# tsadja/ShaSTA

Hardware: AMD Instinct MI355X
Metric: affinity frame-pairs/sec at N=M=500, F=256 (higher is better)
Workload: dtype f32; 1 GPU; synthetic N=M=500, F=256 (num_point 4 x C 64), nf=7: affinity forward from HBM-resident NHWC BEV maps (SURVEY 8a rows 4-16); max_obj=500, num_feats=7, num_point=4, arithmetic=f16x2, parallelism=replica x1

## Files before the change

### shasta_amd/csrc/anchor_split.hip

```cpp
#include "stages.hpp"
#include "lds_dma.hpp"
#include "pieces.hpp"

#include <stdlib.h>

#include <type_traits>

namespace shasta {

struct RowMaxArgs {
    const float* base[4];
    long stride;
    int rows, len;
    unsigned* out;
    float* sumabs;
};
__global__ __launch_bounds__(256) void row_max_kernel(RowMaxArgs a) {
    __shared__ float red[4];
    const int row = blockIdx.y, src = blockIdx.z;
    const int n4 = a.len / 4, per = (n4 + gridDim.x - 1) / gridDim.x;
    const int beg = blockIdx.x * per, end = min(n4, beg + per);
    const f32x4* p = reinterpret_cast<const f32x4*>(a.base[src] + (size_t)row * a.stride);
    float m = 0.0f, sa = 0.0f;
    for (int i = beg + threadIdx.x; i < end; i += 256) {
        const f32x4 v = __builtin_nontemporal_load(p + i);
        m = fmaxf(fmaxf(m, fmaxf(fabsf(v[0]), fabsf(v[1]))), fmaxf(fabsf(v[2]), fabsf(v[3])));
        sa += (fabsf(v[0]) + fabsf(v[1])) + (fabsf(v[2]) + fabsf(v[3]));
    }
#pragma unroll
    for (int off = 32; off > 0; off >>= 1) m = fmaxf(m, __shfl_xor(m, off, 64));
    if ((threadIdx.x & 63) == 0) red[threadIdx.x >> 6] = m;
    __syncthreads();
    if (threadIdx.x == 0) atomicMax(a.out + src * a.rows + row, __float_as_uint(fmaxf(fmaxf(red[0], red[1]), fmaxf(red[2], red[3]))));
    if (a.sumabs) {
        sa = wave_sum(sa);
        if ((threadIdx.x & 63) == 0) atomicAdd(a.sumabs + src * a.rows + row, sa);
    }
}

__global__ __launch_bounds__(256) void aux_ratio_kernel(const unsigned* __restrict__ wmax, const float* __restrict__ sumabs, int rows, int K,
                                                        float* __restrict__ summary) {
    __shared__ float rbest[4];
    __shared__ int ibest[4];
    float best = 0.0f;
    int where = 0;
    for (int r = threadIdx.x; r < rows; r += 256) {
        const float mx = __uint_as_float(wmax[r]), sa = sumabs[r], rest = sa - mx;
        const float ratio = !(mx > 0.0f) || K < 2 ? (mx == mx ? 0.0f : mx) : rest > sa * 1e-6f ? mx * (float)(K - 1) / rest : INFINITY;
        if (!(ratio <= best)) {
            best = ratio;
            where = r;
        }
    }
#pragma unroll
    for (int off = 32; off > 0; off >>= 1) {
        const float ob = __shfl_xor(best, off, 64);
        const int ow = __shfl_xor(where, off, 64);
        if (!(ob <= best)) {
            best = ob;
            where = ow;
        }
    }
    if ((threadIdx.x & 63) == 0) {
        rbest[threadIdx.x >> 6] = best;
        ibest[threadIdx.x >> 6] = where;
    }
    __syncthreads();
    if (threadIdx.x == 0) {
        for (int w = 1; w < 4; ++w)
            if (!(rbest[w] <= best)) {
                best = rbest[w];
                where = ibest[w];
            }
        summary[0] = best;
        summary[1] = (float)where;
    }
}

static int row_max_chunks(int rows, int sources, int len) {
    int c = 1;
    while (c < 64 && rows * sources * c < 2048 && len / (c * 2) >= 4096) c *= 2;
    return c;
}
int launch_x_maxima(const float* feat, const float* prev_feat, int K, int B, int x_batch_stride, unsigned* xmax, hipStream_t st) {
    if (hipMemsetAsync(xmax, 0, (size_t)2 * B * sizeof(unsigned), st) != hipSuccess) return SHASTA_E_LAUNCH;
    RowMaxArgs r;
    r.base[0] = feat;
    r.base[1] = prev_feat;
    r.base[2] = r.base[3] = nullptr;
    r.stride = x_batch_stride;
    r.rows = B;
    r.len = K;
    r.out = xmax;
    r.sumabs = nullptr;
    hipLaunchKernelGGL(row_max_kernel, dim3(row_max_chunks(B, 2, K), B, 2), dim3(256), 0, st, r);
    return check_launch("row_max (activations)");
}
int launch_w_maxima(const float* const W[4], int H, int K, unsigned* wmax, float* sumabs, hipStream_t st) {
    if (hipMemsetAsync(wmax, 0, (size_t)4 * H * sizeof(unsigned), st) != hipSuccess) return SHASTA_E_LAUNCH;
    if (sumabs && hipMemsetAsync(sumabs, 0, ((size_t)4 * H + 16) * sizeof(float), st) != hipSuccess) return SHASTA_E_LAUNCH;
    RowMaxArgs r;
    for (int i = 0; i < 4; ++i) r.base[i] = W[i];
    r.stride = K;
    r.rows = H;
    r.len = K;
    r.out = wmax;
    r.sumabs = sumabs;
    hipLaunchKernelGGL(row_max_kernel, dim3(row_max_chunks(H, 4, K), H, 4), dim3(256), 0, st, r);
    int rc = check_launch("row_max (weights)");
    if (rc || !sumabs) return rc;
    hipLaunchKernelGGL(aux_ratio_kernel, dim3(1), dim3(256), 0, st, wmax, sumabs, 4 * H, K, sumabs + (size_t)4 * H);
    return check_launch("aux_ratio");
}



struct SplitXArgs {
    const float* x[2];
    uint32_t* xs;
    int B, KT, NBLK, XT, x_batch_stride, NP;
    const unsigned* xmax;
};

__global__ __launch_bounds__(256) void split_x_kernel(SplitXArgs a) {
    __shared__ __attribute__((aligned(16))) float tile[32][264];
    const int src = blockIdx.z, bblk = blockIdx.y / a.XT, u = blockIdx.y % a.XT;
    const int kt0 = blockIdx.x * 8, nkt = min(8, a.KT - kt0);
    const float* x = a.x[src];
    const int brow0 = (bblk * a.XT + u) * 32;
    for (int i = threadIdx.x; i < 32 * 64; i += 256) {
        const int r = i >> 6, c4 = i & 63, b = brow0 + r;
        f32x4 v = {0.0f, 0.0f, 0.0f, 0.0f};
        if (b < a.B && (c4 >> 3) < nkt)
            v = *reinterpret_cast<const f32x4*>(x + (size_t)b * a.x_batch_stride + (size_t)kt0 * 32 + c4 * 4);
        *reinterpret_cast<f32x4*>(&tile[r][c4 * 4]) = v;
    }
    __syncthreads();
    for (int i = threadIdx.x; i < 1024; i += 256) {
        const int lane = i & 63, s = (i >> 6) & 1, ktl = i >> 7;
        if (ktl >= nkt) continue;
        const int r = lane & 31, h = lane >> 5;
        const float* p = &tile[r][ktl * 32 + 16 * s + 8 * h];
        const f32x4 v0 = *reinterpret_cast<const f32x4*>(p), v1 = *reinterpret_cast<const f32x4*>(p + 4);
        const float v[8] = {v0[0], v0[1], v0[2], v0[3], v1[0], v1[1], v1[2], v1[3]};
        if (a.NP == 2) {
            const int e = range_exponent_bits(a.xmax[src * a.B + min(brow0 + r, a.B - 1)]);
            u32x4 hi, lo;
            cut2_f16x8([&](int j) { return v[j]; }, e, hi, lo);
            const size_t frag0 = ((((size_t)src * a.NBLK + bblk) * a.KT + kt0 + ktl) * (4 * a.XT)) + (size_t)(u * 2 + s) * 2;
            u32x4* o = reinterpret_cast<u32x4*>(a.xs) + frag0 * 64 + lane;
            o[0] = hi;
            o[64] = lo;
            continue;
        }
        u32x4 hi, mid, lo;
#pragma unroll
        for (int j = 0; j < 4; ++j) {
            float h0, m0, l0, h1, m1, l1;
            cut3_bf16(v[2 * j], h0, m0, l0);
            cut3_bf16(v[2 * j + 1], h1, m1, l1);
            hi[j] = pack_bf16x2(h0, h1);
            mid[j] = pack_bf16x2(m0, m1);
            lo[j] = pack_bf16x2(l0, l1);
        }
        const size_t frag0 = ((((size_t)src * a.NBLK + bblk) * a.KT + kt0 + ktl) * (6 * a.XT)) + (size_t)(u * 2 + s) * 3;
        u32x4* o = reinterpret_cast<u32x4*>(a.xs) + frag0 * 64 + lane;
        o[0] = hi;
        o[64] = mid;
        o[128] = lo;
    }
}

struct PrecutArgs {
    const float* W[4];
    const unsigned* wmax;
    uint32_t* img;
    int H, K, KT, G;
};
__global__ __launch_bounds__(256) void precut_weights_kernel(PrecutArgs a) {
    __shared__ __attribute__((aligned(16))) float tile[32][260];
    const int mlp = blockIdx.z, g = blockIdx.y, kt0 = blockIdx.x * 8, nkt = min(8, a.KT - kt0);
    const float* W = a.W[mlp];
    for (int i = threadIdx.x; i < 32 * 64; i += 256) {
        const int r = i >> 6, c4 = i & 63, row = g * 32 + r;
        f32x4 v = {0.0f, 0.0f, 0.0f, 0.0f};
        if (row < a.H && (c4 >> 3) < nkt) v = __builtin_nontemporal_load(reinterpret_cast<const f32x4*>(W + (size_t)row * a.K + (size_t)kt0 * 32) + c4);
        *reinterpret_cast<f32x4*>(&tile[r][c4 * 4]) = v;
    }
    __syncthreads();
    const int lane = threadIdx.x & 63;
    for (int f = threadIdx.x >> 6; f < 2 * nkt; f += 4) {
        const int ktl = f >> 1, sstep = f & 1;
        const int frow = lane & 31;
        const int wex = range_exponent_bits(a.wmax[mlp * a.H + min(g * 32 + frow, a.H - 1)]);
        const float* p = &tile[frow][ktl * 32 + 16 * sstep + 8 * (lane >> 5)];
        u32x4 hi, lo;
        cut2_f16x8([&](int j) { return p[j]; }, wex, hi, lo);
        u32x4* o = reinterpret_cast<u32x4*>(a.img) + ((((size_t)mlp * a.G + g) * a.KT + kt0 + ktl) * 4 + sstep * 2) * 64 + lane;
        o[0] = hi;
        o[64] = lo;
    }
}
size_t precut_image_bytes(int H, int K) { return (K % 32 != 0 || H == 0) ? 0 : (size_t)4 * cdiv(H, 32) * (K / 32) * 4096; }
int launch_precut_weights(const float* const W[4], const unsigned* wmax, void* img, int H, int K, hipStream_t st) {
    PrecutArgs a;
    for (int i = 0; i < 4; ++i) a.W[i] = W[i];
    a.wmax = wmax;
    a.img = static_cast<uint32_t*>(img);
    a.H = H;
    a.K = K;
    a.KT = K / 32;
    a.G = cdiv(H, 32);
    hipLaunchKernelGGL(precut_weights_kernel, dim3(cdiv(a.KT, 8), a.G, 4), dim3(256), 0, st, a);
    return check_launch("precut_weights");
}

struct AnchorSplitArgs {
    const uint32_t* wimg;
    const float* W[4];
    const uint32_t* xs;
    float* part;
    int H, K, B, KS, Kc, KT, NBLK, groups_per_mlp;
    const unsigned* wmax;
};

template <int XT, int NS, int NP, bool PRECUT = false>
__global__ __launch_bounds__(256) void anchor_l1_split_kernel(AnchorSplitArgs a) {
    static_assert(!PRECUT || NP == 2, "the pre-cut image holds fp16 pieces");
    constexpr int NPROD = NP == 3 ? 6 : 3;
    constexpr int XCH = 2 * NP * XT;
    constexpr int XPW = XCH / 4;
    static_assert(XCH % 4 == 0, "x fragments are dealt to four waves");
    constexpr int SLOT = 4 * 1024 + XCH * 256;
    constexpr int PER_TILE = 4 + XPW;
    static_assert(PER_TILE * (NS - 1) <= 63, "vmcnt is 6 bits");
    constexpr int NM = 2 * NPROD * XT;
    constexpr int ND = PER_TILE;
    constexpr int NR = 4 + XCH;
    constexpr int SG = PRECUT ? 1 : (NM - 8) / 16;
    constexpr int RPG = PRECUT ? (NR + NM - 2) / (NM - 1) : 1;
    static_assert(PRECUT ? (1 + (NR + RPG - 1) / RPG <= NM && 1 + ND <= NM) : (1 + NR < NM && 6 + 15 * SG < NM),
                  "side work must fit the MFMA gaps of one tile");
    extern __shared__ __attribute__((aligned(16))) float lds[];
    const int lane = threadIdx.x & 63;
    const int wid = __builtin_amdgcn_readfirstlane(threadIdx.x >> 6);

    const int ncombo = 2 * a.KS;
    const int combo = blockIdx.x % ncombo, rest = blockIdx.x / ncombo;
    const int quad = rest / a.NBLK;
    const int ks = combo >> 1, src = combo & 1;
    const int G2 = 2 * a.groups_per_mlp;
    const bool active = quad * 4 + wid < G2;
    const int gg = min(quad * 4 + wid, G2 - 1);
    const int mlp = 2 * src + gg / a.groups_per_mlp, r0 = (gg % a.groups_per_mlp) * 32;
    const int bblk = rest % a.NBLK;
    const int tpc = a.Kc >> 5;
    const int kt_beg = ks * tpc, NT = min(a.KT, kt_beg + tpc) - kt_beg;

    const float* wbase = mlp == 0 ? a.W[0] : mlp == 1 ? a.W[1] : mlp == 2 ? a.W[2] : a.W[3];
    const char* wub = PRECUT ? reinterpret_cast<const char*>(a.wimg) + (((size_t)mlp * a.groups_per_mlp + (r0 >> 5)) * a.KT + kt_beg) * 4096
                             : reinterpret_cast<const char*>(wbase + (size_t)r0 * a.K + (size_t)kt_beg * 32);
    const char* xub = reinterpret_cast<const char*>(a.xs) + ((((size_t)src * a.NBLK + bblk) * a.KT + kt_beg) * XCH) * 1024;
    uint32_t woff[4];
    {
        const int cpos = lane & 7, rl = lane >> 3;
#pragma unroll
        for (int j = 0; j < 4; ++j) {
            const int r = 8 * j + rl;
            const int c = cpos ^ ((r >> 1) & 7);
            woff[j] = (uint32_t)(((min(r0 + r, a.H - 1) - r0) * a.K + 4 * c) * 4);
        }
        if (PRECUT) woff[0] = (uint32_t)(lane * 16);
    }
    const uint32_t xoff = (uint32_t)(lane * 16 + wid * 1024);
    const uint32_t lds0 = (uint32_t)(size_t)((__attribute__((address_space(3))) float*)lds);
    auto dma = [&](int t, int slot, int idx) {
        if (idx < 4) {
            const char* base = PRECUT ? wub + (size_t)t * 4096 + (size_t)idx * 1024 : wub + (size_t)t * 128;
            const uint32_t dst = lds0 + (uint32_t)((slot * SLOT + wid * 1024 + idx * 256) * 4);
            lds_dma_x4_nt(PRECUT ? woff[0] : woff[idx], base, dst);
        } else {
            const int i = idx - 4;
            const char* base = xub + (size_t)t * (XCH * 1024) + (size_t)i * 4096;
            const uint32_t dst = lds0 + (uint32_t)((slot * SLOT + 4096 + (wid + 4 * i) * 256) * 4);
            lds_dma_x4(xoff, base, dst);
        }
    };
    auto issue = [&](int t, int slot) {
#pragma unroll
        for (int j = 0; j < ND; ++j) dma(t, slot, j);
    };

    struct Frag {
        u32x4 A[2][NP];
        u32x4 X[XT][2][NP];
    };
    f32x4 raw[4];
    const int frow = lane & 31, fh = lane >> 5, fsw = (frow >> 1) & 7;
    auto read_one = [&](int slot, Frag& f, int idx) {
        const float* sl = lds + slot * SLOT;
        if (idx < 4) {
            const int s = idx >> 1, qq = idx & 1;
            if constexpr (PRECUT) f.A[s][qq] = *reinterpret_cast<const u32x4*>(sl + wid * 1024 + idx * 256 + lane * 4);
            else raw[idx] = *reinterpret_cast<const f32x4*>(sl + wid * 1024 + frow * 32 + (((4 * s + 2 * fh + qq) ^ fsw) * 4));
        } else {
            const int j = idx - 4;
            f.X[j / (2 * NP)][(j / NP) % 2][j % NP] = *reinterpret_cast<const u32x4*>(sl + 4096 + j * 256 + lane * 4);
        }
    };
    float ph = 0.0f, pm = 0.0f, pl = 0.0f;
    _Float16 qh = 0, ql = 0;
    int wex = 0;
    if constexpr (NP == 2 && !PRECUT) wex = range_exponent_bits(a.wmax[mlp * a.H + min(r0 + frow, a.H - 1)]);
    auto cut_one = [&](Frag& f, int e) {
        if constexpr (PRECUT) return;
        const int s = e >> 3, d = (e & 7) >> 1;
        if constexpr (NP == 2) {
            _Float16 h, l;
            cut2_f16(__builtin_ldexpf(raw[e >> 2][e & 3], wex), h, l);
            if ((e & 1) == 0) {
                qh = h;
                ql = l;
            } else {
                f.A[s][0][d] = pack_f16x2(qh, h);
                f.A[s][1][d] = pack_f16x2(ql, l);
            }
        } else {
            float h, m, l;
            cut3_bf16(raw[e >> 2][e & 3], h, m, l);
            if ((e & 1) == 0) {
                ph = h;
                pm = m;
                pl = l;
            } else {
                f.A[s][0][d] = pack_bf16x2(ph, h);
                f.A[s][1][d] = pack_bf16x2(pm, m);
                f.A[s][NP - 1][d] = pack_bf16x2(pl, l);
            }
        }
    };

    f32x16 acc[XT];
#pragma unroll
    for (int u = 0; u < XT; ++u) acc[u] = f32x16{0, 0, 0, 0, 0, 0, 0, 0, 0, 0, 0, 0, 0, 0, 0, 0};
    auto mma_one = [&](const Frag& f, int i) {
        const int s = i / (NPROD * XT), u = (i / NPROD) % XT, pr = i % NPROD;
        if constexpr (NP == 3) acc[u] = mfma_32x32x16_bf16(f.A[s][kProductsBf16[pr].a], f.X[u][s][kProductsBf16[pr].b], acc[u]);
        else acc[u] = mfma_32x32x16_f16(f.A[s][kProductsF16[pr].a], f.X[u][s][kProductsF16[pr].b], acc[u]);
    };

    {
        int s = 0;
#pragma unroll 1
        for (int t = 0; t < NS && t < NT; ++t, ++s) issue(t, s);
    }
    Frag fa, fb;
    if (NT >= NS) wait_vmcnt<PER_TILE*(NS - 1)>();
    else wait_vmcnt<0>();
    __builtin_amdgcn_s_barrier();
    if (NT > 0) {
#pragma unroll
        for (int i = 0; i < NR; ++i) read_one(0, fa, i);
#pragma unroll
        for (int e = 0; e < 16; ++e) cut_one(fa, e);
    }
    auto step = [&](const Frag& cur, Frag& nxt, int t, int sc, auto steady) {
        constexpr bool STEADY = decltype(steady)::value;
        const int sn = sc + 1 == NS ? 0 : sc + 1;
#pragma unroll
        for (int i = 0; i < NM; ++i) {
            mma_one(cur, i);
            __builtin_amdgcn_sched_barrier(0);
            if (i == 0) {
                asm volatile("s_waitcnt lgkmcnt(0)" ::: "memory");
                if constexpr (STEADY) wait_vmcnt<PER_TILE*(NS - 2)>();
                else wait_vmcnt<0>();
                __builtin_amdgcn_s_barrier();
                if constexpr (!STEADY) {
                    if (t + NS < NT) issue(t + NS, sc);
                }
            }
            if (i >= 1 && i - 1 < ND) {
                if constexpr (STEADY) dma(t + NS, sc, i - 1);
            }
            if (i >= 1) {
#pragma unroll
                for (int r = 0; r < RPG; ++r)
                    if ((i - 1) * RPG + r < NR) read_one(sn, nxt, (i - 1) * RPG + r);
            }
            if constexpr (!PRECUT) {
                if (i >= 6 && (i - 6) % SG == 0 && (i - 6) / SG < 16) cut_one(nxt, (i - 6) / SG);
            }
            __builtin_amdgcn_sched_barrier(0);
        }
    };
    int t = 0, sc = 0;
    auto next = [&](int s) { return s + 1 == NS ? 0 : s + 1; };
#pragma unroll 1
    for (; t + NS + 1 < NT; t += 2) {
        step(fa, fb, t, sc, std::true_type{});
        sc = next(sc);
        step(fb, fa, t + 1, sc, std::true_type{});
        sc = next(sc);
    }
#pragma unroll 1
    for (; t + 1 < NT; t += 2) {
        step(fa, fb, t, sc, std::false_type{});
        sc = next(sc);
        step(fb, fa, t + 1, sc, std::false_type{});
        sc = next(sc);
    }
    if (t < NT) step(fa, fb, t, sc, std::false_type{});

    if (active) {
#pragma unroll
        for (int u = 0; u < XT; ++u) {
            const int b = (bblk * XT + u) * 32 + frow;
            if (b < a.B) {
                float* o = a.part + ((size_t)ks * a.B + b) * (4 * a.H) + mlp * a.H;
#pragma unroll
                for (int r = 0; r < 16; ++r) {
                    const int row = r0 + (r & 3) + 8 * (r >> 2) + 4 * fh;
                    if (row < a.H) o[row] = acc[u][r];
                }
            }
        }
    }
}

template <int NS>
__global__ __launch_bounds__(512) void anchor_l1_wide_kernel(AnchorSplitArgs a) {
    constexpr int XT = 16;
    constexpr int SLOT = (8 + 2 * XT) * 256;
    constexpr int ND = 5, NR = 12, NM = 24;
    static_assert(ND * (NS - 1) <= 63, "vmcnt is 6 bits");
    extern __shared__ __attribute__((aligned(16))) float lds[];
    const int lane = threadIdx.x & 63;
    const int wid = __builtin_amdgcn_readfirstlane(threadIdx.x >> 6);
    const int rg2 = wid & 1, ig = wid >> 1;

    const int ncombo = 2 * a.KS;
    const int combo = blockIdx.x % ncombo, rest = blockIdx.x / ncombo;
    const int quad = rest / a.NBLK, bblk = rest % a.NBLK;
    const int ks = combo >> 1, src = combo & 1;
    const int G2 = 2 * a.groups_per_mlp;
    const int tpc = a.Kc >> 5;
    const int kt_beg = ks * tpc, NT = 2 * (min(a.KT, kt_beg + tpc) - kt_beg);

    auto group_base = [&](int gq, int& mlp, int& r0) {
        const int gg = min(quad * 4 + gq, G2 - 1);
        mlp = 2 * src + gg / a.groups_per_mlp;
        r0 = (gg % a.groups_per_mlp) * 32;
    };
    int mlpw, r0w;
    group_base(wid >> 1, mlpw, r0w);
    const char* wub = reinterpret_cast<const char*>(a.wimg) + (((size_t)mlpw * a.groups_per_mlp + (r0w >> 5)) * a.KT + kt_beg) * 4096 + (wid & 1) * 1024;
    const char* xub = reinterpret_cast<const char*>(a.xs) + ((((size_t)src * a.NBLK + bblk) * a.KT + kt_beg) * (4 * XT)) * 1024;
    const uint32_t loff = (uint32_t)(lane * 16);
    const uint32_t lds0 = (uint32_t)(size_t)((__attribute__((address_space(3))) float*)lds);
    auto dma = [&](int t, int slot, int idx) {
        if (idx == 0) {
            const char* base = wub + (size_t)(t >> 1) * 4096 + (size_t)(t & 1) * 2048;
            const uint32_t dst = lds0 + (uint32_t)((slot * SLOT + wid * 256) * 4);
            lds_dma_x4(loff, base, dst);
        } else {
            const int f = 4 * wid + idx - 1, u = f >> 1, pc = f & 1;
            const char* base = xub + (size_t)(t >> 1) * (4 * XT * 1024) + (size_t)(((u * 2 + (t & 1)) * 2 + pc) * 1024);
            const uint32_t dst = lds0 + (uint32_t)((slot * SLOT + 2048 + f * 256) * 4);
            lds_dma_x4(loff, base, dst);
        }
    };
    struct Frag {
        u32x4 A[2][2];
        u32x4 X[4][2];
    };
    auto read_one = [&](int slot, Frag& f, int idx) {
        const float* sl = lds + slot * SLOT + lane * 4;
        if (idx < 4) f.A[idx >> 1][idx & 1] = *reinterpret_cast<const u32x4*>(sl + ((2 * rg2 + (idx >> 1)) * 2 + (idx & 1)) * 256);
        else f.X[(idx - 4) >> 1][idx & 1] = *reinterpret_cast<const u32x4*>(sl + 2048 + ((4 * ig + ((idx - 4) >> 1)) * 2 + (idx & 1)) * 256);
    };
    f32x16 acc[2][4];
#pragma unroll
    for (int j = 0; j < 2; ++j)
#pragma unroll
        for (int u = 0; u < 4; ++u) acc[j][u] = f32x16{0, 0, 0, 0, 0, 0, 0, 0, 0, 0, 0, 0, 0, 0, 0, 0};
    auto mma_one = [&](const Frag& f, int i) {
        const int pr = i >> 3, j = (i >> 2) & 1, u = i & 3;
        acc[j][u] = mfma_32x32x16_f16(f.A[j][kProductsF16[pr].a], f.X[u][kProductsF16[pr].b], acc[j][u]);
    };
    {
        int sl = 0;
#pragma unroll 1
        for (int t = 0; t < NS && t < NT; ++t, ++sl)
#pragma unroll
            for (int j = 0; j < ND; ++j) dma(t, sl, j);
    }
    Frag fa, fb;
    if (NT >= NS) wait_vmcnt<ND*(NS - 1)>();
    else wait_vmcnt<0>();
    __builtin_amdgcn_s_barrier();
    if (NT > 0) {
#pragma unroll
        for (int i = 0; i < NR; ++i) read_one(0, fa, i);
    }
    auto step = [&](const Frag& cur, Frag& nxt, int t, int sc, auto steady) {
        constexpr bool STEADY = decltype(steady)::value;
        const int sn = sc + 1 == NS ? 0 : sc + 1;
#pragma unroll
        for (int i = 0; i < NM; ++i) {
            mma_one(cur, i);
            __builtin_amdgcn_sched_barrier(0);
            if (i == 0) {
                asm volatile("s_waitcnt lgkmcnt(0)" ::: "memory");
                if constexpr (STEADY) wait_vmcnt<ND*(NS - 2)>();
                else wait_vmcnt<0>();
                __builtin_amdgcn_s_barrier();
                if constexpr (!STEADY) {
                    if (t + NS < NT) {
#pragma unroll
                        for (int j = 0; j < ND; ++j) dma(t + NS, sc, j);
                    }
                }
            }
            if (i >= 1 && i - 1 < ND) {
                if constexpr (STEADY) dma(t + NS, sc, i - 1);
            }
            if (i >= 1 && i - 1 < NR) read_one(sn, nxt, i - 1);
            __builtin_amdgcn_sched_barrier(0);
        }
    };
    int t = 0, sc = 0;
    auto next = [&](int s) { return s + 1 == NS ? 0 : s + 1; };
#pragma unroll 1
    for (; t + NS + 1 < NT; t += 2) {
        step(fa, fb, t, sc, std::true_type{});
        sc = next(sc);
        step(fb, fa, t + 1, sc, std::true_type{});
        sc = next(sc);
    }
#pragma unroll 1
    for (; t + 1 < NT; t += 2) {
        step(fa, fb, t, sc, std::false_type{});
        sc = next(sc);
        step(fb, fa, t + 1, sc, std::false_type{});
        sc = next(sc);
    }
    if (t < NT) step(fa, fb, t, sc, std::false_type{});
    const int frow = lane & 31, fh = lane >> 5;
#pragma unroll
    for (int j = 0; j < 2; ++j) {
        if (quad * 4 + 2 * rg2 + j >= G2) continue;
        int mlp, r0;
        group_base(2 * rg2 + j, mlp, r0);
#pragma unroll
        for (int u = 0; u < 4; ++u) {
            const int b = (bblk * XT + 4 * ig + u) * 32 + frow;
            if (b >= a.B) continue;
            float* o = a.part + ((size_t)ks * a.B + b) * (4 * a.H) + mlp * a.H;
#pragma unroll
            for (int r = 0; r < 16; ++r) {
                const int row = r0 + (r & 3) + 8 * (r >> 2) + 4 * fh;
                if (row < a.H) o[row] = acc[j][u][r];
            }
        }
    }
}

static inline bool split_wide(int B, int np, bool precut) { return np == 2 && precut && B > 256 && cdiv(B, 512) * 512 <= cdiv(B, 256) * 256; }

static inline int split_xt(int B, int np) { return np == 2 ? (B > 128 ? 8 : B > 64 ? 4 : B > 32 ? 2 : 1) : (B <= 64 ? 2 : 4); }
static inline int split_nblk(int B, int np) { return cdiv(B, 32 * split_xt(B, np)); }

size_t anchor_split_workspace_bytes(int B, int K) {
    if (B < 2 || K % 32 != 0) return 0;
    const size_t b3 = (size_t)2 * split_nblk(B, 3) * 32 * split_xt(B, 3) * (size_t)K * 6;
    const size_t b2 = (size_t)2 * split_nblk(B, 2) * 32 * split_xt(B, 2) * (size_t)K * 4;
    return align_up(b3 > b2 ? b3 : b2, 256);
}

bool anchor_split_serves(int B, int K, int x_batch_stride) { return B > 32 && K % 32 == 0 && (x_batch_stride & 3) == 0; }

void launch_split_x(const float* feat, const float* prev_feat, void* xs, int K, int B, int x_batch_stride, int np, const unsigned* xmax,
                    bool precut, hipStream_t st) {
    const bool wide = split_wide(B, np, precut);
    const int XT = wide ? 16 : split_xt(B, np), NBLK = wide ? cdiv(B, 512) : split_nblk(B, np), KT = K / 32;
    SplitXArgs sx;
    sx.x[0] = feat;
    sx.x[1] = prev_feat;
    sx.xs = static_cast<uint32_t*>(xs);
    sx.B = B;
    sx.KT = KT;
    sx.NBLK = NBLK;
    sx.XT = XT;
    sx.x_batch_stride = x_batch_stride;
    sx.NP = np;
    sx.xmax = xmax;
    hipLaunchKernelGGL(split_x_kernel, dim3(cdiv(KT, 8), NBLK * XT, 2), dim3(256), 0, st, sx);
}

void launch_anchor_l1_split(const float* const W[4], const void* xs, float* part, int H, int K, int B, int* ks_out, int np,
                            const unsigned* wmax, const void* wimg, hipStream_t st) {
    const bool wide = split_wide(B, np, wimg != nullptr);
    const int XT = wide ? 16 : split_xt(B, np), NBLK = wide ? cdiv(B, 512) : split_nblk(B, np), KT = K / 32;
    AnchorSplitArgs a;
    for (int i = 0; i < 4; ++i) a.W[i] = W[i];
    a.xs = static_cast<const uint32_t*>(xs);
    a.part = part;
    a.H = H;
    a.K = K;
    a.B = B;
    a.KT = KT;
    a.NBLK = NBLK;
    a.groups_per_mlp = cdiv(H, 32);
    a.wmax = wmax;
    a.wimg = static_cast<const uint32_t*>(wimg);
    const int quads = cdiv(2 * a.groups_per_mlp, 4);
    int ncu = 256;
    {
        int dev = 0;
        if (hipGetDevice(&dev) == hipSuccess) {
            int v = 0;
            if (hipDeviceGetAttribute(&v, hipDeviceAttributeMultiprocessorCount, dev) == hipSuccess && v > 0) ncu = v;
        }
    }
    const int cmin = KT >= 64 ? 4 : 1;
    int ks = cmin;
    double best = -1.0;
    const int nblk_split = split_nblk(B, np);
    for (int c = cmin; c <= 64 && c * 16 <= KT; ++c) {
        const int wgs = 2 * cdiv(KT, cdiv(KT, c)) * quads * nblk_split;
        const int rounds = cdiv(wgs, ncu);
        const double eff = (double)wgs / ((double)rounds * ncu);
        if (eff > best + 1e-9) {
            best = eff;
            ks = c;
        }
    }
    const int tiles_per = cdiv(KT, ks);
    a.Kc = tiles_per * 32;
    a.KS = cdiv(KT, tiles_per);
    *ks_out = a.KS;
    auto launch = [&](auto kern, int ns, int xt) {
        const size_t ldsb = (size_t)ns * (4 * 1024 + 2 * np * xt * 256) * sizeof(float);
        (void)hipFuncSetAttribute((const void*)kern, hipFuncAttributeMaxDynamicSharedMemorySize, (int)ldsb);
        hipLaunchKernelGGL(kern, dim3(2 * a.KS * quads * NBLK), dim3(256), ldsb, st, a);
    };
    if (wide) {
        const size_t ldsb = (size_t)4 * (8 + 2 * 16) * 1024;
        if (hipFuncSetAttribute((const void*)anchor_l1_wide_kernel<4>, hipFuncAttributeMaxDynamicSharedMemorySize, (int)ldsb) == hipSuccess) {
            hipLaunchKernelGGL(anchor_l1_wide_kernel<4>, dim3(2 * a.KS * quads * NBLK), dim3(512), ldsb, st, a);
        } else {
            (void)hipGetLastError();
            const size_t lds3 = (size_t)3 * (8 + 2 * 16) * 1024;
            (void)hipFuncSetAttribute((const void*)anchor_l1_wide_kernel<3>, hipFuncAttributeMaxDynamicSharedMemorySize, (int)lds3);
            hipLaunchKernelGGL(anchor_l1_wide_kernel<3>, dim3(2 * a.KS * quads * NBLK), dim3(512), lds3, st, a);
        }
    } else if (np == 2 && wimg) {
        if (XT == 1) launch(anchor_l1_split_kernel<1, 6, 2, true>, 6, 1);
        else if (XT == 2) launch(anchor_l1_split_kernel<2, 5, 2, true>, 5, 2);
        else if (XT == 4) launch(anchor_l1_split_kernel<4, 4, 2, true>, 4, 4);
        else launch(anchor_l1_split_kernel<8, 3, 2, true>, 3, 8);
    } else if (np == 2) {
        if (XT == 4) launch(anchor_l1_split_kernel<4, 4, 2>, 4, 4);
        else launch(anchor_l1_split_kernel<8, 3, 2>, 3, 8);
    } else if (XT == 2) launch(anchor_l1_split_kernel<2, 5, 3>, 5, 2);
    else launch(anchor_l1_split_kernel<4, 4, 3>, 4, 4);
}

}
```

Measured before the change: 64630 frame-pairs/s.

## Load activation fragments directly to registers in wide anchor kernel, stage only weights in LDS

The wide anchor layer-1 kernel previously staged both weight and activation tiles through LDS via DMA. Now each wave loads its own activation fragments straight from global memory into registers one step ahead, and only the shared weight tiles go through LDS. The wave-to-tile mapping changes from a 2x4 to a 4x2 accumulator layout, the LDS ring shrinks to 3 small slots, and the output store uses 16-byte vector writes when aligned. This cuts LDS footprint and LDS traffic, but exposes global-load latency directly to registers with only one step of prefetch and raises register pressure.

```diff
diff --git a/shasta_amd/csrc/anchor_split.hip b/shasta_amd/csrc/anchor_split.hip
--- a/shasta_amd/csrc/anchor_split.hip
+++ b/shasta_amd/csrc/anchor_split.hip
@@ -428,16 +428,21 @@
     }
 }
 
+
+template <int OFF>
+__device__ __forceinline__ void global_load_x4(u32x4& dst, uint32_t voff, const char* base) {
+    asm volatile("global_load_dwordx4 %0, %1, %2 offset:%3" : "=&v"(dst) : "v"(voff), "s"(base), "n"(OFF) : "memory");
+}
+
 template <int NS>
 __global__ __launch_bounds__(512) void anchor_l1_wide_kernel(AnchorSplitArgs a) {
     constexpr int XT = 16;
-    constexpr int SLOT = (8 + 2 * XT) * 256;
-    constexpr int ND = 5, NR = 12, NM = 24;
-    static_assert(ND * (NS - 1) <= 63, "vmcnt is 6 bits");
+    constexpr int SLOT = 8 * 256;
+    constexpr int NX = 4, NR = 8, NM = 24;
+    static_assert(NS >= 3, "the DMA of step t + NS may still be in flight when step t + 1 is read");
     extern __shared__ __attribute__((aligned(16))) float lds[];
     const int lane = threadIdx.x & 63;
     const int wid = __builtin_amdgcn_readfirstlane(threadIdx.x >> 6);
-    const int rg2 = wid & 1, ig = wid >> 1;
 
     const int ncombo = 2 * a.KS;
     const int combo = blockIdx.x % ncombo, rest = blockIdx.x / ncombo;
@@ -455,48 +460,46 @@
     int mlpw, r0w;
     group_base(wid >> 1, mlpw, r0w);
     const char* wub = reinterpret_cast<const char*>(a.wimg) + (((size_t)mlpw * a.groups_per_mlp + (r0w >> 5)) * a.KT + kt_beg) * 4096 + (wid & 1) * 1024;
-    const char* xub = reinterpret_cast<const char*>(a.xs) + ((((size_t)src * a.NBLK + bblk) * a.KT + kt_beg) * (4 * XT)) * 1024;
-    const uint32_t loff = (uint32_t)(lane * 16);
+    const char* xub = reinterpret_cast<const char*>(a.xs) + ((((size_t)src * a.NBLK + bblk) * a.KT + kt_beg) * (4 * XT) + 8 * wid) * 1024;
+    const uint32_t loff = (uint32_t)(lane * 16), loff1 = loff + 4096;
     const uint32_t lds0 = (uint32_t)(size_t)((__attribute__((address_space(3))) float*)lds);
-    auto dma = [&](int t, int slot, int idx) {
-        if (idx == 0) {
-            const char* base = wub + (size_t)(t >> 1) * 4096 + (size_t)(t & 1) * 2048;
-            const uint32_t dst = lds0 + (uint32_t)((slot * SLOT + wid * 256) * 4);
-            lds_dma_x4(loff, base, dst);
-        } else {
-            const int f = 4 * wid + idx - 1, u = f >> 1, pc = f & 1;
-            const char* base = xub + (size_t)(t >> 1) * (4 * XT * 1024) + (size_t)(((u * 2 + (t & 1)) * 2 + pc) * 1024);
-            const uint32_t dst = lds0 + (uint32_t)((slot * SLOT + 2048 + f * 256) * 4);
-            lds_dma_x4(loff, base, dst);
-        }
+    auto dma = [&](int t, int slot) {
+        const char* base = wub + (size_t)(t >> 1) * 4096 + (size_t)(t & 1) * 2048;
+        const uint32_t dst = lds0 + (uint32_t)((slot * SLOT + wid * 256) * 4);
+        lds_dma_x4(loff, base, dst);
     };
     struct Frag {
-        u32x4 A[2][2];
-        u32x4 X[4][2];
+        u32x4 A[4][2];
+        u32x4 X[2][2];
+    };
+    auto load_x = [&](int t, Frag& f, int idx) {
+        const char* base = xub + (size_t)(t >> 1) * (4 * XT * 1024) + (size_t)(t & 1) * 2048;
+        if (idx & 1) global_load_x4<1024>(f.X[idx >> 1][1], idx >> 1 ? loff1 : loff, base);
+        else global_load_x4<0>(f.X[idx >> 1][0], idx >> 1 ? loff1 : loff, base);
     };
     auto read_one = [&](int slot, Frag& f, int idx) {
-        const float* sl = lds + slot * SLOT + lane * 4;
-        if (idx < 4) f.A[idx >> 1][idx & 1] = *reinterpret_cast<const u32x4*>(sl + ((2 * rg2 + (idx >> 1)) * 2 + (idx & 1)) * 256);
-        else f.X[(idx - 4) >> 1][idx & 1] = *reinterpret_cast<const u32x4*>(sl + 2048 + ((4 * ig + ((idx - 4) >> 1)) * 2 + (idx & 1)) * 256);
-    };
-    f32x16 acc[2][4];
-#pragma unroll
-    for (int j = 0; j < 2; ++j)
-#pragma unroll
-        for (int u = 0; u < 4; ++u) acc[j][u] = f32x16{0, 0, 0, 0, 0, 0, 0, 0, 0, 0, 0, 0, 0, 0, 0, 0};
+        f.A[idx >> 1][idx & 1] = *reinterpret_cast<const u32x4*>(lds + slot * SLOT + idx * 256 + lane * 4);
+    };
+    f32x16 acc[4][2];
+#pragma unroll
+    for (int j = 0; j < 4; ++j)
+#pragma unroll
+        for (int u = 0; u < 2; ++u) acc[j][u] = f32x16{0, 0, 0, 0, 0, 0, 0, 0, 0, 0, 0, 0, 0, 0, 0, 0};
     auto mma_one = [&](const Frag& f, int i) {
-        const int pr = i >> 3, j = (i >> 2) & 1, u = i & 3;
+        const int pr = i >> 3, j = (i >> 1) & 3, u = i & 1;
         acc[j][u] = mfma_32x32x16_f16(f.A[j][kProductsF16[pr].a], f.X[u][kProductsF16[pr].b], acc[j][u]);
     };
+    Frag fa, fb;
+    if (NT > 0) {
+#pragma unroll
+        for (int i = 0; i < NX; ++i) load_x(0, fa, i);
+    }
     {
         int sl = 0;
 #pragma unroll 1
-        for (int t = 0; t < NS && t < NT; ++t, ++sl)
-#pragma unroll
-            for (int j = 0; j < ND; ++j) dma(t, sl, j);
-    }
-    Frag fa, fb;
-    if (NT >= NS) wait_vmcnt<ND*(NS - 1)>();
+        for (int t = 0; t < NS && t < NT; ++t, ++sl) dma(t, sl);
+    }
+    if (NT >= NS) wait_vmcnt<NS - 2>();
     else wait_vmcnt<0>();
     __builtin_amdgcn_s_barrier();
     if (NT > 0) {
@@ -512,20 +515,19 @@
             __builtin_amdgcn_sched_barrier(0);
             if (i == 0) {
                 asm volatile("s_waitcnt lgkmcnt(0)" ::: "memory");
-                if constexpr (STEADY) wait_vmcnt<ND*(NS - 2)>();
+                __builtin_amdgcn_s_barrier();
+            }
+            if (i >= 1 && i - 1 < NX) {
+                if (STEADY || t + 1 < NT) load_x(t + 1, nxt, i - 1);
+            }
+            if (i == 1 + NX) {
+                if (STEADY || t + NS < NT) dma(t + NS, sc);
+            }
+            if (i >= 2 + NX && i - 2 - NX < NR) read_one(sn, nxt, i - 2 - NX);
+            if (i == NM - 1) {
+                if constexpr (STEADY) wait_vmcnt<1>();
                 else wait_vmcnt<0>();
-                __builtin_amdgcn_s_barrier();
-                if constexpr (!STEADY) {
-                    if (t + NS < NT) {
-#pragma unroll
-                        for (int j = 0; j < ND; ++j) dma(t + NS, sc, j);
-                    }
-                }
-            }
-            if (i >= 1 && i - 1 < ND) {
-                if constexpr (STEADY) dma(t + NS, sc, i - 1);
-            }
-            if (i >= 1 && i - 1 < NR) read_one(sn, nxt, i - 1);
+            }
             __builtin_amdgcn_sched_barrier(0);
         }
     };
@@ -547,20 +549,27 @@
     }
     if (t < NT) step(fa, fb, t, sc, std::false_type{});
     const int frow = lane & 31, fh = lane >> 5;
-#pragma unroll
-    for (int j = 0; j < 2; ++j) {
-        if (quad * 4 + 2 * rg2 + j >= G2) continue;
+    const bool vec = (a.H & 3) == 0 && (reinterpret_cast<uintptr_t>(a.part) & 15) == 0;
+#pragma unroll
+    for (int j = 0; j < 4; ++j) {
+        if (quad * 4 + j >= G2) continue;
         int mlp, r0;
-        group_base(2 * rg2 + j, mlp, r0);
-#pragma unroll
-        for (int u = 0; u < 4; ++u) {
-            const int b = (bblk * XT + 4 * ig + u) * 32 + frow;
+        group_base(j, mlp, r0);
+#pragma unroll
+        for (int u = 0; u < 2; ++u) {
+            const int b = (bblk * XT + 2 * wid + u) * 32 + frow;
             if (b >= a.B) continue;
             float* o = a.part + ((size_t)ks * a.B + b) * (4 * a.H) + mlp * a.H;
 #pragma unroll
-            for (int r = 0; r < 16; ++r) {
-                const int row = r0 + (r & 3) + 8 * (r >> 2) + 4 * fh;
-                if (row < a.H) o[row] = acc[j][u][r];
+            for (int q = 0; q < 4; ++q) {
+                const int row = r0 + 8 * q + 4 * fh;
+                if (vec) {
+                    if (row < a.H) *reinterpret_cast<f32x4*>(o + row) = f32x4{acc[j][u][4 * q], acc[j][u][4 * q + 1], acc[j][u][4 * q + 2], acc[j][u][4 * q + 3]};
+                } else {
+#pragma unroll
+                    for (int r = 0; r < 4; ++r)
+                        if (row + r < a.H) o[row + r] = acc[j][u][4 * q + r];
+                }
             }
         }
     }
@@ -646,15 +655,8 @@
         hipLaunchKernelGGL(kern, dim3(2 * a.KS * quads * NBLK), dim3(256), ldsb, st, a);
     };
     if (wide) {
-        const size_t ldsb = (size_t)4 * (8 + 2 * 16) * 1024;
-        if (hipFuncSetAttribute((const void*)anchor_l1_wide_kernel<4>, hipFuncAttributeMaxDynamicSharedMemorySize, (int)ldsb) == hipSuccess) {
-            hipLaunchKernelGGL(anchor_l1_wide_kernel<4>, dim3(2 * a.KS * quads * NBLK), dim3(512), ldsb, st, a);
-        } else {
-            (void)hipGetLastError();
-            const size_t lds3 = (size_t)3 * (8 + 2 * 16) * 1024;
-            (void)hipFuncSetAttribute((const void*)anchor_l1_wide_kernel<3>, hipFuncAttributeMaxDynamicSharedMemorySize, (int)lds3);
-            hipLaunchKernelGGL(anchor_l1_wide_kernel<3>, dim3(2 * a.KS * quads * NBLK), dim3(512), lds3, st, a);
-        }
+        constexpr int NSW = 3;
+        hipLaunchKernelGGL(anchor_l1_wide_kernel<NSW>, dim3(2 * a.KS * quads * NBLK), dim3(512), (size_t)NSW * 8192, st, a);
     } else if (np == 2 && wimg) {
         if (XT == 1) launch(anchor_l1_split_kernel<1, 6, 2, true>, 6, 1);
         else if (XT == 2) launch(anchor_l1_split_kernel<2, 5, 2, true>, 5, 2);
```

After: 60200 frame-pairs/s. 6.8% lower.
